# heracles-ec/heracles

Measured on AMD Instinct MI355X. Metric: map->Cl pairs/sec + mixing-matrix build sec, nside=4096 lmax=6144, higher is better.
Workload: dtype f64

## Files before the change

heracles_amd/csrc/hx_twopoint.hip:

```cpp
#include <algorithm>

#include "hx_common.h"

namespace hx {

constexpr int CL_T = 6;
constexpr int CL_TW = 8;
constexpr int CL_LB = 64;
constexpr int CL_SYNC = 8;

struct ClTile {
    int i0, j0;
    int out[CL_T * CL_T];
};

__global__ __launch_bounds__(CL_TW * 64) void k_alm2cl_rows(
    const double2 *const *__restrict__ comp, const int *__restrict__ comp_lmax, int ncomp,
    const ClTile *__restrict__ tiles, int ntiles, int ngroups, int nmsplit, int lmax_out, int nlblk, double *__restrict__ part, long long part_stride,
    int m_lo, int m_hi, int m_step)
{
    const int nq = nlblk * nmsplit;
    const int q = ((int)blockIdx.x / (8 * ngroups)) * 8 + ((int)blockIdx.x & 7), g = ((int)blockIdx.x >> 3) % ngroups;
    if (q >= nq) return;
    const int ms = q % nmsplit, lblk = nlblk - 1 - q / nmsplit;
    const int lane = threadIdx.x & 63, w = threadIdx.x >> 6;
    const int ti = g * CL_TW + w;
    const bool have = ti < ntiles;
    const ClTile tile = tiles[have ? ti : 0];
    const int l = lblk * CL_LB + lane;
    const int lhi = min(lblk * CL_LB + CL_LB - 1, lmax_out);
    const double2 *pa[CL_T], *pb[CL_T];
    long long La[CL_T], Lb[CL_T];
#pragma unroll
    for (int t = 0; t < CL_T; ++t) {
        int ia = min(tile.i0 + t, ncomp - 1), ib = min(tile.j0 + t, ncomp - 1);
        pa[t] = comp[ia]; La[t] = comp_lmax[ia];
        pb[t] = comp[ib]; Lb[t] = comp_lmax[ib];
    }
    double acc[CL_T * CL_T];
#pragma unroll
    for (int t = 0; t < CL_T * CL_T; ++t) acc[t] = 0.0;
    const int mend = min(lhi, m_hi - 1);
    int k = 0;
    for (int m = m_lo + ms * m_step; m <= mend; m += nmsplit * m_step, ++k) {
        if (have && m <= l && l <= lmax_out) {
            double2 a[CL_T], b[CL_T];
#pragma unroll
            for (int t = 0; t < CL_T; ++t) {
                a[t] = l <= La[t] ? pa[t][(long long)m * (2 * La[t] + 1 - m) / 2 + l] : make_double2(0.0, 0.0);
                b[t] = l <= Lb[t] ? pb[t][(long long)m * (2 * Lb[t] + 1 - m) / 2 + l] : make_double2(0.0, 0.0);
            }
            const double wgt = m == 0 ? 1.0 : 2.0;
#pragma unroll
            for (int s = 0; s < CL_T; ++s)
#pragma unroll
                for (int t = 0; t < CL_T; ++t) {
                    double p = a[s].x * b[t].x;
                    if (m != 0) p = fma(a[s].y, b[t].y, p);
                    acc[s * CL_T + t] = fma(wgt, p, acc[s * CL_T + t]);
                }
        }
        if ((k & (CL_SYNC - 1)) == CL_SYNC - 1) __syncthreads();
    }
    if (have && l <= lmax_out) {
#pragma unroll
        for (int t = 0; t < CL_T * CL_T; ++t) {
            const int o = tile.out[t];
            if (o >= 0) part[(long long)ms * part_stride + (long long)o * (lmax_out + 1) + l] = acc[t];
        }
    }
}

__global__ __launch_bounds__(256) void k_alm2cl_finish(const double *__restrict__ part, long long part_stride, int nmsplit, long long n, int lmax_out,
                                                        double *__restrict__ cls)
{
    const long long i = (long long)blockIdx.x * blockDim.x + threadIdx.x;
    if (i >= n) return;
    double s = 0.0;
    for (int q = 0; q < nmsplit; ++q) s += part[(long long)q * part_stride + i];
    cls[i] = s / (2.0 * (double)(i % (lmax_out + 1)) + 1.0);
}

}

using namespace hx;

namespace hx {
struct Alm2clScratch {
    DevBuf ptrs, lmax, tiles, part, out;
};
static Alm2clScratch *g_alm2cl_scratch = nullptr;
static Alm2clScratch &alm2cl_scratch()
{
    if (!g_alm2cl_scratch) g_alm2cl_scratch = new Alm2clScratch;
    return *g_alm2cl_scratch;
}
void alm2cl_drop_cache()
{
    if (!g_alm2cl_scratch) return;
    g_alm2cl_scratch->ptrs.release(); g_alm2cl_scratch->lmax.release(); g_alm2cl_scratch->tiles.release();
    g_alm2cl_scratch->part.release(); g_alm2cl_scratch->out.release();
}
}

extern "C" int hx_alm2cl_pairs_range(int ncomp, const int *lmax_i, const double *const *alms, int lmax_out, int npairs, const int *pair_i,
                                     const int *pair_j, int m0, int m1, int mstep, double *cls);

extern "C" int hx_alm2cl_pairs(int ncomp, const int *lmax_i, const double *const *alms,
                               int lmax_out, int npairs, const int *pair_i, const int *pair_j,
                               double *cls)
{
    return hx_alm2cl_pairs_range(ncomp, lmax_i, alms, lmax_out, npairs, pair_i, pair_j, 0, lmax_out + 1, 1, cls);
}

extern "C" int hx_alm2cl_pairs_range(int ncomp, const int *lmax_i, const double *const *alms, int lmax_out, int npairs, const int *pair_i,
                                     const int *pair_j, int m0, int m1, int mstep, double *cls)
{
    HX_TRY(ensure_ready());
    if (m0 < 0 || m1 < m0 || mstep < 1) return fail(HX_ERR_ARG, "hx_alm2cl_pairs_range: bad orders %d, %d + %d, ... < %d", m0, m0, mstep, m1);
    if (ncomp <= 0 || npairs < 0 || !lmax_i || !alms || !pair_i || !pair_j || !cls || lmax_out < 0)
        return fail(HX_ERR_ARG, "hx_alm2cl_pairs: bad argument");
    if (npairs == 0) return HX_OK;
    for (int c = 0; c < ncomp; ++c)
        if (!alms[c] || lmax_i[c] < 0) return fail(HX_ERR_ARG, "hx_alm2cl_pairs: component %d invalid", c);
    for (int p = 0; p < npairs; ++p) {
        if (pair_i[p] < 0 || pair_i[p] >= ncomp || pair_j[p] < 0 || pair_j[p] >= ncomp)
            return fail(HX_ERR_ARG, "hx_alm2cl_pairs: pair %d out of range", p);
        if (lmax_i[pair_i[p]] < lmax_out || lmax_i[pair_j[p]] < lmax_out)
            return fail(HX_ERR_ARG, "hx_alm2cl_pairs: lmax_out exceeds lmax of pair %d", p);
    }
    hipStream_t st = rt().stream;

    std::vector<InView> views(ncomp);
    std::vector<const double2 *> ptrs(ncomp);
    for (int c = 0; c < ncomp; ++c) {
        size_t nlm = (size_t)(lmax_i[c] + 1) * (lmax_i[c] + 2) / 2;
        HX_TRY(views[c].bind(alms[c], nlm * sizeof(double2)));
        ptrs[c] = views[c].as<double2>();
    }
    const int nb = (ncomp + CL_T - 1) / CL_T;
    std::map<std::pair<int, int>, int> tile_of;
    std::vector<ClTile> tiles;
    for (int p = 0; p < npairs; ++p) {
        int ci = pair_i[p], cj = pair_j[p];
        if (ci / CL_T > cj / CL_T) std::swap(ci, cj);
        int bi = ci / CL_T, bj = cj / CL_T;
        auto key = std::make_pair(bi, bj);
        auto it = tile_of.find(key);
        if (it == tile_of.end()) {
            ClTile t;
            t.i0 = bi * CL_T;
            t.j0 = bj * CL_T;
            for (int k = 0; k < CL_T * CL_T; ++k) t.out[k] = -1;
            tiles.push_back(t);
            it = tile_of.emplace(key, (int)tiles.size() - 1).first;
        }
        ClTile &t = tiles[it->second];
        int slot = (ci - t.i0) * CL_T + (cj - t.j0);
        if (t.out[slot] >= 0) {
            ClTile d;
            d.i0 = t.i0; d.j0 = t.j0;
            for (int k = 0; k < CL_T * CL_T; ++k) d.out[k] = -1;
            d.out[slot] = p;
            tiles.push_back(d);
        } else
            t.out[slot] = p;
    }
    (void)nb;
    std::stable_sort(tiles.begin(), tiles.end(), [](const ClTile &x, const ClTile &y) { return x.i0 != y.i0 ? x.i0 < y.i0 : x.j0 < y.j0; });
    Alm2clScratch &sc_ = alm2cl_scratch();
    DevBuf &d_ptrs = sc_.ptrs, &d_lmax = sc_.lmax, &d_tiles = sc_.tiles;
    HX_TRY(d_ptrs.alloc(sizeof(void *) * ncomp));
    HX_TRY(d_lmax.alloc(sizeof(int) * ncomp));
    HX_TRY(d_tiles.alloc(sizeof(ClTile) * tiles.size()));
    HX_HIP(hipMemcpyAsync(d_ptrs.p, ptrs.data(), sizeof(void *) * ncomp, hipMemcpyHostToDevice, st));
    HX_HIP(hipMemcpyAsync(d_lmax.p, lmax_i, sizeof(int) * ncomp, hipMemcpyHostToDevice, st));
    HX_HIP(hipMemcpyAsync(d_tiles.p, tiles.data(), sizeof(ClTile) * tiles.size(), hipMemcpyHostToDevice, st));
    const size_t out_bytes = sizeof(double) * (size_t)npairs * (lmax_out + 1);
    double *out_dev = cls;
    const bool out_on_host = !is_device_ptr(cls);
    if (out_on_host) {
        HX_TRY(sc_.out.alloc(out_bytes));
        out_dev = sc_.out.as<double>();
    }

    const int nlblk = (lmax_out + CL_LB) / CL_LB;
    const int ngroups = ((int)tiles.size() + CL_TW - 1) / CL_TW;
    int nmsplit = (int)((2.5 * rt().cus) / ((double)nlblk * ngroups) + 0.5);
    nmsplit = std::max(1, std::min(nmsplit, 8));
    const long long nout = (long long)npairs * (lmax_out + 1);
    DevBuf &d_part = sc_.part;
    HX_TRY(d_part.alloc(sizeof(double) * (size_t)nout * nmsplit));
    HX_HIP(hipMemsetAsync(d_part.p, 0, sizeof(double) * (size_t)nout * nmsplit, st));
    {
        ProfScope ps("alm2cl");
        hipLaunchKernelGGL(k_alm2cl_rows, dim3((unsigned)((nlblk * nmsplit + 7) / 8 * 8 * ngroups)), dim3(CL_TW * 64), 0, st,
                           d_ptrs.as<const double2 *>(), d_lmax.as<int>(), ncomp, d_tiles.as<ClTile>(), (int)tiles.size(), ngroups, nmsplit,
                           lmax_out, nlblk, d_part.as<double>(), nout, m0, m1, mstep);
        hipLaunchKernelGGL(k_alm2cl_finish, dim3((unsigned)((nout + 255) / 256)), dim3(256), 0, st, d_part.as<double>(), nout, nmsplit, nout,
                           lmax_out, out_dev);
    }
    HX_HIP(hipGetLastError());
    if (out_on_host) HX_TRY(copy_d2h(cls, out_dev, out_bytes));
    HX_HIP(hipStreamSynchronize(st));
    if (sc_.part.bytes + sc_.out.bytes > ((size_t)512 << 20)) alm2cl_drop_cache();
    return HX_OK;
}

namespace hx {
__global__ __launch_bounds__(256) void k_alm_resample(int lmax_in, int lmax_out, long long nlm_in, long long nlm_out,
                                                      const double2 *__restrict__ in, double2 *__restrict__ out)
{
    const int m = blockIdx.x;
    const double2 *src = in + (long long)blockIdx.y * nlm_in;
    double2 *dst = out + (long long)blockIdx.y * nlm_out;
    const long long bo = (long long)m * (2 * lmax_out + 1 - m) / 2, bi = (long long)m * (2 * lmax_in + 1 - m) / 2;
    for (int l = m + threadIdx.x; l <= lmax_out; l += blockDim.x)
        dst[bo + l] = (m <= lmax_in && l <= lmax_in) ? src[bi + l] : make_double2(0.0, 0.0);
}
}

extern "C" int hx_alm_resample(int lmax_in, int lmax_out, int ncomp, const double *alm_in, double *alm_out)
{
    using namespace hx;
    HX_TRY(ensure_ready());
    if (lmax_in < 0 || lmax_out < 0 || ncomp < 0 || (ncomp > 0 && (!alm_in || !alm_out)))
        return fail(HX_ERR_ARG, "hx_alm_resample: bad arguments");
    if (ncomp == 0) return HX_OK;
    const long long ni = (long long)(lmax_in + 1) * (lmax_in + 2) / 2, no = (long long)(lmax_out + 1) * (lmax_out + 2) / 2;
    InView vin;
    OutView vout;
    HX_TRY(vin.bind(alm_in, sizeof(double2) * ni * ncomp));
    HX_TRY(vout.bind(alm_out, sizeof(double2) * no * ncomp));
    hipLaunchKernelGGL(k_alm_resample, dim3(lmax_out + 1, ncomp), dim3(256), 0, rt().stream, lmax_in, lmax_out, ni, no,
                       vin.as<double2>(), vout.as<double2>());
    HX_HIP(hipGetLastError());
    HX_TRY(vout.finish());
    return finish_call();
}


namespace hx {
struct SubList {
    const double2 *p[4];
};
__global__ __launch_bounds__(256) void k_alm_subtract(long long n, const double2 *__restrict__ full, int nsub, SubList subs,
                                                      double2 *__restrict__ out)
{
    long long i = (long long)blockIdx.x * blockDim.x + threadIdx.x;
    const long long st = (long long)gridDim.x * blockDim.x;
    for (; i < n; i += st) {
        double2 v = full[i];
        for (int k = 0; k < nsub; ++k) {
            const double2 s = subs.p[k][i];
            v.x -= s.x;
            v.y -= s.y;
        }
        out[i] = v;
    }
}

__global__ __launch_bounds__(256) void k_region_maps(long long npix, int ncomp, const double *__restrict__ maps,
                                                     const double *__restrict__ region, double k, double *__restrict__ out)
{
    long long i = (long long)blockIdx.x * blockDim.x + threadIdx.x;
    const long long st = (long long)gridDim.x * blockDim.x;
    for (; i < npix; i += st) {
        const bool in = region[i] == k;
        for (int c = 0; c < ncomp; ++c) out[(long long)c * npix + i] = in ? maps[(long long)c * npix + i] : 0.0;
    }
}
}

extern "C" int hx_alm_subtract(int64_t n, const double *full, int nsub, const double *const *subs, double *out)
{
    using namespace hx;
    HX_TRY(ensure_ready());
    if (n < 0 || nsub < 0 || nsub > 4 || (n > 0 && (!full || !out || (nsub > 0 && !subs))))
        return fail(HX_ERR_ARG, "hx_alm_subtract: bad arguments (at most 4 arrays to subtract)");
    if (n == 0) return HX_OK;
    InView vf, vs[4];
    OutView vo;
    HX_TRY(vf.bind(full, sizeof(double2) * n));
    SubList sl;
    for (int k = 0; k < 4; ++k) sl.p[k] = nullptr;
    for (int k = 0; k < nsub; ++k) {
        if (!subs[k]) return fail(HX_ERR_ARG, "hx_alm_subtract: null array %d", k);
        HX_TRY(vs[k].bind(subs[k], sizeof(double2) * n));
        sl.p[k] = vs[k].as<double2>();
    }
    HX_TRY(vo.bind(out, sizeof(double2) * n));
    hipLaunchKernelGGL(k_alm_subtract, dim3(4096), dim3(256), 0, rt().stream, (long long)n, vf.as<double2>(), nsub, sl, vo.as<double2>());
    HX_HIP(hipGetLastError());
    HX_TRY(vo.finish());
    HX_HIP(hipStreamSynchronize(rt().stream));
    return HX_OK;
}

extern "C" int hx_region_maps(int64_t npix, int ncomp, const double *maps, const double *region, double k, double *out)
{
    using namespace hx;
    HX_TRY(ensure_ready());
    if (npix < 0 || ncomp < 0 || (npix > 0 && ncomp > 0 && (!maps || !region || !out))) return fail(HX_ERR_ARG, "hx_region_maps: bad arguments");
    if (npix == 0 || ncomp == 0) return HX_OK;
    InView vm, vr;
    OutView vo;
    HX_TRY(vm.bind(maps, sizeof(double) * npix * ncomp));
    HX_TRY(vr.bind(region, sizeof(double) * npix));
    HX_TRY(vo.bind(out, sizeof(double) * npix * ncomp));
    hipLaunchKernelGGL(k_region_maps, dim3(4096), dim3(256), 0, rt().stream, (long long)npix, ncomp, vm.as<double>(), vr.as<double>(), k, vo.as<double>());
    HX_HIP(hipGetLastError());
    HX_TRY(vo.finish());
    HX_HIP(hipStreamSynchronize(rt().stream));
    return HX_OK;
}
```

Baseline: 428.7.

## Add alm2cl kernel that stages each alm row once in LDS via async loads

Adds a new alm-to-Cl kernel, used when all components share the same lmax. It groups up to 16 tiles over at most 10 component blocks, loads each needed alm row into LDS once per m using global_load_lds with a multi-stage ring buffer, and has each wave compute two 6x6 tiles from LDS. The aim is to cut redundant global reads of the same rows across tiles and to overlap loads with FMA work. It costs up to 160KB of LDS per block, which lowers occupancy, and relies on inline GCN assembly and a hand-built vmcnt wait scheme. The old tile kernel remains as a fallback, selectable with an environment variable.

After: 429.7 (median of 6 runs). Within noise of the previous version (+0.2%).

```diff
diff --git a/heracles_amd/csrc/hx_twopoint.hip b/heracles_amd/csrc/hx_twopoint.hip
--- a/heracles_amd/csrc/hx_twopoint.hip
+++ b/heracles_amd/csrc/hx_twopoint.hip
@@ -1,4 +1,6 @@
 #include <algorithm>
+#include <cstdlib>
+#include <cstring>
 
 #include "hx_common.h"
 
@@ -71,6 +73,153 @@
     }
 }
 
+constexpr int CL1_TILES = 2 * CL_TW;
+constexpr int CL1_BLKS = 10;
+constexpr int CL1_ROWS = CL1_BLKS * CL_T;
+constexpr int CL1_LPW = (CL1_ROWS + 7) / 8;
+constexpr int CL1_LDS = 160 * 1024;
+
+struct ClOnceTile {
+    int sa, sb;
+    int out[CL_T * CL_T];
+};
+struct ClOnceGroup {
+    int tile0, ntiles;
+    int nrows;
+    int comp[CL1_ROWS];
+    int row[CL1_ROWS];
+};
+
+__device__ __forceinline__ void cl_glds16(const double2 *sbase, unsigned voff_bytes, unsigned lds_dst)
+{
+    unsigned keep;
+    asm volatile("s_mov_b32 %0, m0\n\ts_mov_b32 m0, %3\n\ts_nop 2\n\tglobal_load_lds_dwordx4 %1, %2\n\ts_mov_b32 m0, %0"
+                 : "=&s"(keep)
+                 : "v"(voff_bytes), "s"(sbase), "s"(lds_dst)
+                 : "memory");
+}
+__device__ __forceinline__ void cl_wait_loads(int n)
+{
+#define HX_CL_W(N) case N: asm volatile("s_waitcnt vmcnt(" #N ")" ::: "memory"); break;
+    switch (n) {
+        HX_CL_W(1) HX_CL_W(2) HX_CL_W(3) HX_CL_W(4) HX_CL_W(5) HX_CL_W(6) HX_CL_W(7) HX_CL_W(8) HX_CL_W(9) HX_CL_W(10) HX_CL_W(12)
+        HX_CL_W(14) HX_CL_W(15) HX_CL_W(16) HX_CL_W(18) HX_CL_W(21) HX_CL_W(24)
+    default: asm volatile("s_waitcnt vmcnt(0)" ::: "memory"); break;
+    }
+#undef HX_CL_W
+}
+
+template <bool M0>
+__device__ __forceinline__ void cl_tile_order(const double2 *__restrict__ ra, const double2 *__restrict__ rb, double wgt, double (&acc)[CL_T * CL_T])
+{
+    double2 a[CL_T], b[CL_T];
+#pragma unroll
+    for (int t = 0; t < CL_T; ++t) {
+        a[t] = ra[t * CL_LB];
+        b[t] = rb[t * CL_LB];
+    }
+#pragma unroll
+    for (int s = 0; s < CL_T; ++s)
+#pragma unroll
+        for (int t = 0; t < CL_T; ++t) {
+            double p = a[s].x * b[t].x;
+            if (!M0) p = fma(a[s].y, b[t].y, p);
+            acc[s * CL_T + t] = fma(wgt, p, acc[s * CL_T + t]);
+        }
+}
+
+__global__ __launch_bounds__(CL_TW * 64) void k_alm2cl_once(
+    const double2 *const *__restrict__ comp, int L, const ClOnceGroup *__restrict__ groups, const ClOnceTile *__restrict__ tiles, int ngroups,
+    int nmsplit, int lmax_out, int nlblk, double *__restrict__ part, long long part_stride, int m_lo, int m_hi, int m_step, int stage_rows,
+    int nst)
+{
+    extern __shared__ __align__(16) unsigned char cl_lds[];
+    const int q = (int)blockIdx.x / ngroups, g = (int)blockIdx.x % ngroups;
+    const int ms = q % nmsplit, lblk = nlblk - 1 - q / nmsplit;
+    const int lane = threadIdx.x & 63;
+    const int w = __builtin_amdgcn_readfirstlane((int)threadIdx.x >> 6);
+    const ClOnceGroup &grp = groups[g];
+    const int l = lblk * CL_LB + lane;
+    const int lhi = min(lblk * CL_LB + CL_LB - 1, lmax_out);
+    const int nrows = grp.nrows;
+    const int lpw = (nrows - w + 7) >> 3;
+    const double2 *rp[CL1_LPW];
+    unsigned rl[CL1_LPW];
+    const unsigned lds0 = (unsigned)(unsigned long long)(const __attribute__((address_space(3))) void *)cl_lds;
+#pragma unroll
+    for (int j = 0; j < CL1_LPW; ++j) {
+        const int r = min(w + 8 * j, nrows - 1);
+        rp[j] = comp[grp.comp[r]];
+        rl[j] = lds0 + (unsigned)grp.row[r] * (CL_LB * (unsigned)sizeof(double2));
+    }
+    const bool have0 = w < grp.ntiles, have1 = w + CL_TW < grp.ntiles;
+    const ClOnceTile *t0 = tiles + grp.tile0 + (have0 ? w : 0), *t1 = tiles + grp.tile0 + (have1 ? w + CL_TW : 0);
+    const int sa0 = t0->sa, sb0 = t0->sb, sa1 = t1->sa, sb1 = t1->sb;
+    double acc0[CL_T * CL_T], acc1[CL_T * CL_T];
+#pragma unroll
+    for (int t = 0; t < CL_T * CL_T; ++t) acc0[t] = acc1[t] = 0.0;
+    const int mend = min(lhi, m_hi - 1);
+    const int mfirst = m_lo + ms * m_step, mstride = nmsplit * m_step;
+    const int nk = mfirst <= mend ? (mend - mfirst) / mstride + 1 : 0;
+    const unsigned stage_bytes = (unsigned)stage_rows * (CL_LB * (unsigned)sizeof(double2));
+    const int lc = min(l, lmax_out);
+    double one = 1.0, two = 2.0;
+    asm volatile("" : "+v"(one), "+v"(two));
+
+    int m_iss = mfirst, st_iss = 0, k_iss = 0;
+#define HX_CL_ISSUE()                                                                                                                     \
+    do {                                                                                                                                  \
+        const long long rb_ = (long long)m_iss * (2 * (long long)L + 1 - m_iss) / 2;                                                      \
+        const unsigned vo_ = (unsigned)max(lc, m_iss) * (unsigned)sizeof(double2);                                                        \
+        const unsigned so_ = (unsigned)st_iss * stage_bytes;                                                                              \
+        _Pragma("unroll") for (int j_ = 0; j_ < CL1_LPW; ++j_)                                                                            \
+            if (j_ < lpw) cl_glds16(rp[j_] + rb_, vo_, rl[j_] + so_);                                                                     \
+        m_iss += mstride; ++k_iss;                                                                                                        \
+        if (++st_iss == nst) st_iss = 0;                                                                                                  \
+    } while (0)
+    while (k_iss < nst - 1 && k_iss < nk) HX_CL_ISSUE();
+    int m = mfirst, st = 0, k = 0;
+#define HX_CL_STEP(M0)                                                                                                                    \
+    do {                                                                                                                                  \
+                                       \
+        cl_wait_loads(min(nst - 2, nk - 1 - k) * lpw);                                                                                    \
+        asm volatile("s_waitcnt lgkmcnt(0)" ::: "memory");      \
+        __builtin_amdgcn_s_barrier();                                                                                                     \
+        if (k_iss < nk) HX_CL_ISSUE();                                                                 \
+        if (m <= l && l <= lmax_out) {                                                                                                    \
+            const double2 *ls_ = reinterpret_cast<const double2 *>(cl_lds + (unsigned)st * stage_bytes) + lane;                           \
+                           \
+            cl_tile_order<M0>(ls_ + sa0 * CL_LB, ls_ + sb0 * CL_LB, M0 ? one : two, acc0);                                                \
+            __builtin_amdgcn_sched_barrier(0);                                                                                            \
+            cl_tile_order<M0>(ls_ + sa1 * CL_LB, ls_ + sb1 * CL_LB, M0 ? one : two, acc1);                                                \
+            __builtin_amdgcn_sched_barrier(0);                                                                                            \
+        }                                                                                                                                 \
+        if (++st == nst) st = 0;                                                                                                          \
+        ++k; m += mstride;                                                                                                                \
+    } while (0)
+    if (nk > 0 && mfirst == 0) HX_CL_STEP(true);
+    while (k < nk) HX_CL_STEP(false);
+#undef HX_CL_STEP
+#undef HX_CL_ISSUE
+    if (l <= lmax_out) {
+        double *dst = part + (long long)ms * part_stride + l;
+        if (have0) {
+#pragma unroll
+            for (int t = 0; t < CL_T * CL_T; ++t) {
+                const int o = t0->out[t];
+                if (o >= 0) dst[(long long)o * (lmax_out + 1)] = acc0[t];
+            }
+        }
+        if (have1) {
+#pragma unroll
+            for (int t = 0; t < CL_T * CL_T; ++t) {
+                const int o = t1->out[t];
+                if (o >= 0) dst[(long long)o * (lmax_out + 1)] = acc1[t];
+            }
+        }
+    }
+}
+
 __global__ __launch_bounds__(256) void k_alm2cl_finish(const double *__restrict__ part, long long part_stride, int nmsplit, long long n, int lmax_out,
                                                         double *__restrict__ cls)
 {
@@ -87,7 +236,7 @@
 
 namespace hx {
 struct Alm2clScratch {
-    DevBuf ptrs, lmax, tiles, part, out;
+    DevBuf ptrs, lmax, tiles, groups, part, out;
 };
 static Alm2clScratch *g_alm2cl_scratch = nullptr;
 static Alm2clScratch &alm2cl_scratch()
@@ -99,7 +248,7 @@
 {
     if (!g_alm2cl_scratch) return;
     g_alm2cl_scratch->ptrs.release(); g_alm2cl_scratch->lmax.release(); g_alm2cl_scratch->tiles.release();
-    g_alm2cl_scratch->part.release(); g_alm2cl_scratch->out.release();
+    g_alm2cl_scratch->groups.release(); g_alm2cl_scratch->part.release(); g_alm2cl_scratch->out.release();
 }
 }
 
@@ -171,11 +320,7 @@
     Alm2clScratch &sc_ = alm2cl_scratch();
     DevBuf &d_ptrs = sc_.ptrs, &d_lmax = sc_.lmax, &d_tiles = sc_.tiles;
     HX_TRY(d_ptrs.alloc(sizeof(void *) * ncomp));
-    HX_TRY(d_lmax.alloc(sizeof(int) * ncomp));
-    HX_TRY(d_tiles.alloc(sizeof(ClTile) * tiles.size()));
     HX_HIP(hipMemcpyAsync(d_ptrs.p, ptrs.data(), sizeof(void *) * ncomp, hipMemcpyHostToDevice, st));
-    HX_HIP(hipMemcpyAsync(d_lmax.p, lmax_i, sizeof(int) * ncomp, hipMemcpyHostToDevice, st));
-    HX_HIP(hipMemcpyAsync(d_tiles.p, tiles.data(), sizeof(ClTile) * tiles.size(), hipMemcpyHostToDevice, st));
     const size_t out_bytes = sizeof(double) * (size_t)npairs * (lmax_out + 1);
     double *out_dev = cls;
     const bool out_on_host = !is_device_ptr(cls);
@@ -192,7 +337,60 @@
     DevBuf &d_part = sc_.part;
     HX_TRY(d_part.alloc(sizeof(double) * (size_t)nout * nmsplit));
     HX_HIP(hipMemsetAsync(d_part.p, 0, sizeof(double) * (size_t)nout * nmsplit, st));
-    {
+    bool once = true;
+    for (int c = 1; c < ncomp; ++c) once = once && lmax_i[c] == lmax_i[0];
+    if (const char *e = getenv("HX_ALM2CL_KERNEL")) once = once && strcmp(e, "tiles") != 0;
+    std::vector<ClOnceGroup> groups;
+    std::vector<ClOnceTile> otiles;
+    if (once) {
+        otiles.resize(tiles.size());
+        int stage_rows = 0;
+        for (size_t t = 0; t < tiles.size();) {
+            ClOnceGroup G;
+            std::vector<int> blks;
+            auto slot = [&blks](int b) { return (int)(std::find(blks.begin(), blks.end(), b) - blks.begin()); };
+            G.tile0 = (int)t;
+            for (; t < tiles.size() && (int)t - G.tile0 < CL1_TILES; ++t) {
+                const int bi = tiles[t].i0 / CL_T, bj = tiles[t].j0 / CL_T;
+                const size_t more = (slot(bi) == (int)blks.size()) + (bj != bi && slot(bj) == (int)blks.size());
+                if (blks.size() + more > (size_t)CL1_BLKS) break;
+                if (slot(bi) == (int)blks.size()) blks.push_back(bi);
+                if (slot(bj) == (int)blks.size()) blks.push_back(bj);
+                otiles[t].sa = slot(bi) * CL_T;
+                otiles[t].sb = slot(bj) * CL_T;
+                std::copy(tiles[t].out, tiles[t].out + CL_T * CL_T, otiles[t].out);
+            }
+            G.ntiles = (int)t - G.tile0;
+            G.nrows = 0;
+            for (int r = 0; r < CL1_ROWS; ++r) G.comp[r] = G.row[r] = 0;
+            for (size_t s = 0; s < blks.size(); ++s)
+                for (int c = blks[s] * CL_T; c < std::min(blks[s] * CL_T + CL_T, ncomp); ++c) {
+                    G.comp[G.nrows] = c;
+                    G.row[G.nrows++] = (int)s * CL_T + (c - blks[s] * CL_T);
+                }
+            stage_rows = std::max(stage_rows, (int)blks.size() * CL_T);
+            groups.push_back(G);
+        }
+        const int nst = std::min(5, CL1_LDS / (stage_rows * CL_LB * (int)sizeof(double2)));
+        const size_t lds = (size_t)nst * stage_rows * CL_LB * sizeof(double2);
+        HX_HIP(hipFuncSetAttribute(reinterpret_cast<const void *>(k_alm2cl_once), hipFuncAttributeMaxDynamicSharedMemorySize, CL1_LDS));
+        HX_TRY(sc_.groups.alloc(sizeof(ClOnceGroup) * groups.size()));
+        HX_TRY(d_tiles.alloc(sizeof(ClOnceTile) * otiles.size()));
+        HX_HIP(hipMemcpyAsync(sc_.groups.p, groups.data(), sizeof(ClOnceGroup) * groups.size(), hipMemcpyHostToDevice, st));
+        HX_HIP(hipMemcpyAsync(d_tiles.p, otiles.data(), sizeof(ClOnceTile) * otiles.size(), hipMemcpyHostToDevice, st));
+        {
+            ProfScope ps("alm2cl");
+            hipLaunchKernelGGL(k_alm2cl_once, dim3((unsigned)(nlblk * nmsplit * (int)groups.size())), dim3(CL_TW * 64), lds, st,
+                               d_ptrs.as<const double2 *>(), lmax_i[0], sc_.groups.as<ClOnceGroup>(), d_tiles.as<ClOnceTile>(), (int)groups.size(),
+                               nmsplit, lmax_out, nlblk, d_part.as<double>(), nout, m0, m1, mstep, stage_rows, nst);
+            hipLaunchKernelGGL(k_alm2cl_finish, dim3((unsigned)((nout + 255) / 256)), dim3(256), 0, st, d_part.as<double>(), nout, nmsplit, nout,
+                               lmax_out, out_dev);
+        }
+    } else {
+        HX_TRY(d_lmax.alloc(sizeof(int) * ncomp));
+        HX_TRY(d_tiles.alloc(sizeof(ClTile) * tiles.size()));
+        HX_HIP(hipMemcpyAsync(d_lmax.p, lmax_i, sizeof(int) * ncomp, hipMemcpyHostToDevice, st));
+        HX_HIP(hipMemcpyAsync(d_tiles.p, tiles.data(), sizeof(ClTile) * tiles.size(), hipMemcpyHostToDevice, st));
         ProfScope ps("alm2cl");
         hipLaunchKernelGGL(k_alm2cl_rows, dim3((unsigned)((nlblk * nmsplit + 7) / 8 * 8 * ngroups)), dim3(CL_TW * 64), 0, st,
                            d_ptrs.as<const double2 *>(), d_lmax.as<int>(), ncomp, d_tiles.as<ClTile>(), (int)tiles.size(), ngroups, nmsplit,
```
